# matt-graham/auxiliary-pm-mcmc

Measured on AMD Instinct MI355X. Metric: MCMC iters/sec + ESS/sec on θ, GP-classif N=4096 N_imp=256, 1/2/4/8 GPU, higher is better.
Workload: dtype mixed f64/f32

## Files before the change

### auxiliary-pm-mcmc_amd/csrc/apm_host.h

```cpp
#pragma once
#include <hip/hip_runtime.h>

#include <algorithm>
#include <cstdint>
#include <cstring>
#include <functional>
#include <initializer_list>
#include <map>
#include <string>
#include <tuple>
#include <utility>
#include <vector>

#include "../../include/apm.h"
#include "apm_internal.h"

#define HIPC(x)                                                                              \
    do {                                                                                     \
        hipError_t e_ = (x);                                                                 \
        if (e_ != hipSuccess)                                                                \
            throw HipError{std::string(#x) + ": " + hipGetErrorString(e_)};                  \
    } while (0)

namespace apm_host __attribute__((visibility("hidden"))) {

struct ProfRec {
    hipEvent_t a, b;
    int kind;
    double work;
};

#define APM_ICM_Q 1.0e3

struct Edges {
    hipEvent_t gram_k = nullptr;
    hipEvent_t cholk_done = nullptr;
    hipEvent_t y2 = nullptr;
    hipEvent_t bottom_done = nullptr;
    std::vector<hipEvent_t> cholk_rel;
    std::vector<hipEvent_t> lp_panel;
    std::vector<hipEvent_t> df;
    std::vector<hipEvent_t> far;
    std::vector<hipEvent_t*> all() {
        std::vector<hipEvent_t*> v{&gram_k, &cholk_done, &y2, &bottom_done};
        for (auto* w : {&cholk_rel, &lp_panel, &df, &far})
            for (hipEvent_t& e : *w) v.push_back(&e);
        return v;
    }
};

typedef std::pair<unsigned*, int> DevList;
typedef std::map<std::tuple<int, int, int, int, int, int>, DevList> ListCache;

struct StagePin {
    int64_t B;
    size_t slots() const { return 0; }
    size_t ubufs() const { return slots() + sizeof(int64_t) * B; }
    size_t h3ok() const { return ubufs() + sizeof(int64_t) * B; }
    size_t h3post() const { return h3ok() + sizeof(int) * B; }
    size_t invok() const { return h3post() + sizeof(int) * B; }
    size_t icm() const { return invok() + 2 * sizeof(int) * B; }
    size_t bytes() const { return icm() + sizeof(double) * B; }
};
enum StageBlk {
    BLK_I3 = 0, BLK_A = 1, BLK_B = 2, BLK_CA = 3, BLK_CB = 4, BLK_SEEDS = 5, BLK_CTRS = 6,
    BLK_FIELDS = 7
};
inline size_t read_back_bytes(int64_t B) { return (sizeof(double) + 3 * sizeof(int)) * B; }

}

struct __attribute__((visibility("hidden"))) apm_ctx {
    int device = 0;
    hipStream_t stream = nullptr;
    int kind = 0, n = 0, d = 0, np = 0, nb = 0, P = 0, S = 0, sp = 0;
    int max_batch = 0, n_slots = 0, n_ubufs = 0;
    static constexpr int outer = 8, outer32 = 8;
    static constexpr int symv_tpw = 2;
    std::vector<int> slot_refs;
    std::vector<int> slot_wide;
    std::vector<int> slot_failed;
    std::vector<double*> l64_h, l64_free;
    double** l64_d = nullptr;
    double eps = 1e-8, tol = 1e-4;
    int lik = APM_LIK_PROBIT;
    int64_t max_iters = 1000;
    std::string err;
    double *X = nullptr, *y = nullptr, *theta = nullptr;
    MatB K{}, A{};
    double *Dinv = nullptr, *ldet = nullptr, *out = nullptr, *partial = nullptr;
    int64_t dstride = 0, lstride = 0, pstride = 0;
    NewtonVecs v{};
    double* vecbase = nullptr;
    double* rvec = nullptr;
    double* sympart = nullptr;
    int64_t sstride = 0;
    bool mixed = true;
    int n_refine = 3;
    double refine_tol = 1e-3;
    int *active = nullptr, *status = nullptr, *n_iter = nullptr;
    int* refining = nullptr;
    double* refine_prev = nullptr;
    int64_t n_refine_steps = 0, n_fp64_rerun = 0;
    int64_t n_icm_check = 0;
    int64_t n_guard = 0;
    double icm_q = APM_ICM_Q;
    int64_t *d_slots = nullptr, *d_ubufs = nullptr, *d_i3 = nullptr;
    char* hpin = nullptr;
    int64_t* hblk = nullptr;
    double* hth = nullptr;
    unsigned* hx = nullptr;
    unsigned* dx = nullptr;
    double *d_ca = nullptr, *d_cb = nullptr;
    uint64_t *d_seeds = nullptr, *d_ctrs = nullptr;
    double* U64 = nullptr;
    SlotSet Sl{};
    UPool Up{};
    std::vector<void*> allocs;
    bool k_full = false;
    int prof = 0;
    std::vector<hipEvent_t> evpool;
    size_t evnext = 0;
    std::vector<apm_host::ProfRec> recs;
    apm_host::ListCache tile_lists, super_lists, super_lists_solo, super_lists_ext;
    std::map<std::tuple<int, int, int, int>, apm_host::DevList> quad_lists;
    bool h3 = true;
// ... 234 lines not shown
```

### auxiliary-pm-mcmc_amd/csrc/apm_internal.h

```cpp
#pragma once
#include <string>

#include "apm_common.h"
#include "tile_lists.h"
#include "tri_index.h"

struct MatB {
    double* base;
    int64_t ld;
    int64_t cstride;
};

struct MatF {
    float* base;
    int64_t ld;
    int64_t cstride;
};

struct Live {
    const int* active;
    int* status;
};
__device__ __forceinline__ bool live_chain(const Live& lv, int b) {
    return lv.active[b] != 0 && lv.status[b] == 0;
// ... 54 lines not shown
                              const int* h3ok, hipStream_t s,
                              Planes16 pl = Planes16{nullptr, 0, 0, 0});

void launch_chol_update32(MatF A, int k0, int kc, const unsigned* tiles, int ntiles, Live live,
                          int nchains, hipStream_t s,
                          FusedDiag<float> fd = FusedDiag<float>{0, nullptr, 0, nullptr, 0, 0},
                          int hlim = 0, const int* h3ok = nullptr);
enum {
    UPD32_NEWTON = 0,
    UPD32_POST = 1,
    UPD32_NEWTON_PLANES = 2,
};
void launch_chol_update32_t128(MatF A, int k0, int kc, const unsigned* tiles, int ntiles,
                               Live live, int nchains, hipStream_t s,
                               FusedDiag<float> fd = FusedDiag<float>{0, nullptr, 0, nullptr, 0, 0},
                               int hlim = 0, const int* h3ok = nullptr, int rhs = -1,
                               int role = UPD32_NEWTON, Planes16 pl = Planes16{nullptr, 0, 0, 0});
void launch_chol_update32_q256(MatF A, int k0, int kc, const unsigned* quads, int nq, Live live,
                               int nchains, hipStream_t s, const int* h3ok, Planes16 pl,
                               int role = UPD32_NEWTON, int npan = 1, int64_t pstep = 0);
void launch_rhs_row_update32(MatF A, int k0, int kc, const unsigned* tiles, int ntiles, Live live,
                             int nchains, hipStream_t s);

void launch_symv(MatB K, const double* x, int64_t xstride, double* y, int64_t ystride,
                 double* part, int64_t pstride, int np, MatF Bf, const double* Ws,
                 int64_t wstride, Live live, int nchains, hipStream_t s, int symv_tpw = 1);
void launch_row32(MatF Bf, int64_t row, int np, double* out, int64_t ostride, Live live,
                  int nchains, hipStream_t s);
void launch_trsv_fwd32(MatF A, int J, int nb, const float* Dinv, int64_t dstride, double* r,
                       double* y, int64_t vstride, Live live, int nchains, hipStream_t s);
void launch_trsv_bwd32(MatF A, int J, const float* Dinv, int64_t dstride, double* r, double* z,
                       int64_t vstride, Live live, int nchains, hipStream_t s);
bool trsv32_mw_ok(int np);
void trsv32_mw_init();
long launch_trsv32_mw(bool fwd, MatF A, int nb, const float* Dinv, int64_t dstride,
                      const double* r, double* out, int64_t vstride, Live live, int nchains,
                      int fail_code, SpinCtl sc, hipStream_t s);
void launch_refine_check(const double* x, const double* d, int64_t vstride, int np, double tol,
                         int fail_code, int step, bool last, double* prev, int* refining,
                         const int* status, int nchains, hipStream_t s);
void launch_refine_mask(Live live, int* refining, int nchains, hipStream_t s);
void launch_refine(int mode, const double* Ws, const double* Kb, double* x, const double* Kt,
                   double* out, int64_t vstride, int np, Live live, int nchains, hipStream_t s);

enum { APM_FAM_SE = 0, APM_FAM_M32 = 1, APM_FAM_M52 = 2 };
struct KernelKind {
    int family;
    int iso;
    int bias;
    bool on_device() const { return family >= 0; }
    int64_t theta_len(int64_t d) const { return family < 0 ? 0 : (iso ? 2 : d + 1) + bias; }
};
inline KernelKind kernel_kind_of(int kind) {
    const int bias = (kind & 16) ? 1 : 0;
    switch (kind & ~16) {
        case 0: return KernelKind{APM_FAM_SE, 1, bias};
        case 1: return KernelKind{APM_FAM_SE, 0, bias};
        case 3: return KernelKind{APM_FAM_M32, 1, bias};
        case 4: return KernelKind{APM_FAM_M32, 0, bias};
        case 5: return KernelKind{APM_FAM_M52, 1, bias};
        case 6: return KernelKind{APM_FAM_M52, 0, bias};
        default: return KernelKind{-1, 0, 0};
    }
// ... 240 lines not shown
```

### auxiliary-pm-mcmc_amd/csrc/host_ctx.cpp

```cpp
#include <cmath>
#include <cstdlib>

#include "apm_host.h"

namespace {
thread_local apm_host::SkewState t_skew;
constexpr int SKEW_US_SECONDARY = 1000, SKEW_US_MAIN = 40;
}

void skew_point(hipStream_t s) {
    if (!t_skew.mode || !s) return;
    if ((t_skew.mode & 1) && (s == t_skew.s2 || s == t_skew.s3))
        launch_delay(SKEW_US_SECONDARY, s);
    else if ((t_skew.mode & 2) && s == t_skew.main)
        launch_delay(SKEW_US_MAIN, s);
}

namespace apm_host {

SkewScope::SkewScope(const apm_ctx* c) : prev(t_skew) {
    t_skew = SkewState{c->skew & 3, c->stream, c->stream2, c->stream3};
}
SkewScope::~SkewScope() { t_skew = prev; }

// ... 87 lines not shown
        c->l64_free.pop_back();
    } else {
        c->l64_h[slot] = dalloc<double>(c, c->np * c->np);
    }
}
void detach_l64(apm_ctx* c, int64_t slot) {
    if (!c->l64_h[slot]) return;
    c->l64_free.push_back(c->l64_h[slot]);
    c->l64_h[slot] = nullptr;
}
void upload_l64(apm_ctx* c) {
    HIPC(hipMemcpyAsync(c->l64_d, c->l64_h.data(), sizeof(double*) * c->n_slots,
                        hipMemcpyHostToDevice, c->stream));
}

void init_ctx(apm_ctx* c, int device, int kind, const double* X, int64_t n, int64_t d,
              int64_t ldx, const double* y, double eps, int64_t S, int64_t max_batch,
              int64_t n_slots, int64_t n_ubufs) {
    c->device = device;
    HIPC(hipSetDevice(device));
    trsv32_mw_init();
    if (const char* e = getenv("APM_MIXED")) c->mixed = atoi(e) != 0;
    if (const char* e = getenv("APM_H3")) c->h3 = atoi(e) != 0;
    if (const char* e = getenv("APM_REFINE_TOL")) c->refine_tol = atof(e);
    if (const char* e = getenv("APM_ICM_Q")) c->icm_q = std::max(0.0, atof(e));
    if (const char* e = getenv("APM_SPIN_LIMIT")) c->spin_df = c->spin_trsv = std::max(1, atoi(e));
    if (const char* e = getenv("APM_SKEW")) c->skew = std::max(0, std::min(7, atoi(e)));
    {
        int least = 0, greatest = 0;
        HIPC(hipDeviceGetStreamPriorityRange(&least, &greatest));
        HIPC(hipStreamCreateWithPriority(&c->stream, hipStreamNonBlocking, greatest));
        HIPC(hipStreamCreateWithPriority(&c->stream2, hipStreamNonBlocking, least));
        HIPC(hipStreamCreateWithPriority(&c->stream3, hipStreamNonBlocking, least));
    }
    c->kind = kind;
    c->n = (int)n;
    c->d = (int)d;
    c->np = (int)((n + 63) / 64 * 64);
    c->nb = c->np / 64;
    {
        const int np64 = (c->nb + c->outer - 1) / c->outer, np32 = (c->nb + c->outer32 - 1) / c->outer32;
        c->ev.cholk_rel.assign(np64, nullptr);
        c->ev.lp_panel.assign(np64, nullptr);
        c->ev.df.assign(np32, nullptr);
        c->ev.far.assign(np32, nullptr);
        for (hipEvent_t* e : c->ev.all()) HIPC(hipEventCreateWithFlags(e, hipEventDisableTiming));
// ... 32 lines not shown
    c->partial = dalloc<double>(c, B * c->pstride);
    const int64_t vs = np;
    c->vecbase = dalloc<double>(c, 8 * B * vs);
    c->rvec = dalloc<double>(c, 3 * B * vs);
    c->sstride = (int64_t)c->nb * c->nb * 64;
    c->sympart = dalloc<double>(c, B * c->sstride);
    c->v = NewtonVecs{c->vecbase,          c->vecbase + 1 * B * vs, c->vecbase + 2 * B * vs,
                      c->vecbase + 3 * B * vs, c->vecbase + 4 * B * vs, c->vecbase + 5 * B * vs,
                      c->vecbase + 6 * B * vs, c->vecbase + 7 * B * vs, vs};
    HIPC(hipMemset(c->vecbase, 0, sizeof(double) * 8 * B * vs));
    c->active = dalloc<int>(c, B);
    c->status = dalloc<int>(c, B);
    c->n_iter = dalloc<int>(c, B);
    c->refining = dalloc<int>(c, B);
    c->active2 = dalloc<int>(c, B);
    c->status2 = dalloc<int>(c, B);
    c->refine_prev = dalloc<double>(c, B);
    c->d_slots = dalloc<int64_t>(c, 2 * B);
    c->d_ubufs = c->d_slots + B;
    HIPC(hipHostMalloc(reinterpret_cast<void**>(&c->hpin), pin_of(c).bytes(),
                       hipHostMallocDefault));
    HIPC(hipHostMalloc(reinterpret_cast<void**>(&c->hmask), sizeof(int) * (size_t)B,
                       hipHostMallocDefault));
    HIPC(hipHostMalloc(reinterpret_cast<void**>(&c->hx), read_back_bytes(B),
                       hipHostMallocMapped | hipHostMallocCoherent));
    HIPC(hipHostGetDevicePointer(reinterpret_cast<void**>(&c->dx), c->hx, 0));
    c->h3ok = dalloc<int>(c, 3 * B);
    c->h3post = c->h3ok + B;
    c->invok = c->h3ok + 2 * B;
    c->guard = dalloc<double>(c, 6 * B);
    HIPC(hipMemset(c->guard, 0, sizeof(double) * 6 * B));
    c->guard_rows = dalloc<double>(c, B * np);
    c->icm_thr = dalloc<double>(c, B);
    if (c->mixed && c->h3) {
        c->plane_cs = 2 * np * 32 * 2 * c->outer32;
        const int npan = (c->nb + c->outer32 - 1) / c->outer32;
        const char* fl = getenv("APM_FAR_LEFT");
        if (npan > 2 && !(fl && atoi(fl) == 0)) {
            void* p = nullptr;
            if (hipMalloc(&p, sizeof(unsigned short) * npan * B * c->plane_cs) == hipSuccess) {
                c->allocs.push_back(p);
                c->planes = static_cast<unsigned short*>(p);
                c->plane_bufs = npan;
                c->far_left = true;
            } else {
                (void)hipGetLastError();
            }
// ... 77 lines not shown
```

### auxiliary-pm-mcmc_amd/csrc/host_newton.cpp

```cpp
#include "apm_host.h"

namespace apm_host {

unsigned long long* spin_words(apm_ctx* c) {
    return c->dfprog + (size_t)c->max_batch * (c->nb + 1);
}
void reset_tickets(apm_ctx* c) {
    HIPC(hipMemsetAsync(spin_words(c) + 2, 0, sizeof(unsigned long long), c->stream));
    c->ticket_base = 0;
}

namespace {

MatF b32_of(apm_ctx* c) {
    return MatF{reinterpret_cast<float*>(c->A.base), c->np, 2 * c->A.cstride};
}
SpinCtl spin_ctl(apm_ctx* c, bool trsv) {
    unsigned long long* w = spin_words(c);
    return SpinCtl{w + 2, c->ticket_base, trsv ? w + 1 : w, trsv ? c->spin_trsv : c->spin_df};
}
void trsv32(apm_ctx* c, bool fwd, MatF F, const float* D, int64_t ds, const double* r,
            double* out, Live lv, int count) {
    c->ticket_base += (unsigned long long)launch_trsv32_mw(
        fwd, F, c->nb, D, ds, r, out, c->v.vstride, lv, count, APM_STATUS_CHOL_B,
        spin_ctl(c, true), c->stream);
}
int64_t plane_step(apm_ctx* c) { return (int64_t)c->max_batch * c->plane_cs; }
Planes16 planes_of(apm_ctx* c, int K) {
    if (!c->planes || !c->h3_now) return Planes16{nullptr, 0, 0, 0};
    return Planes16{c->planes + plane_step(c) * ((K / c->outer32) % c->plane_bufs), c->plane_cs,
                    c->plane_cs / 2, c->np};
}
float* dinv32_of(apm_ctx* c) { return reinterpret_cast<float*>(c->Dinv); }

void tracked_update32(apm_ctx* c, MatF M, int k0, int kc, int i0, int R, int j0, int jend,
                      int count, int fuse_k = -1, int fail_code = 0, hipStream_t st = nullptr,
                      Planes16 pl = Planes16{nullptr, 0, 0, 0}, int jext = -1) {
    if (!st) st = c->stream;
    if (i0 < j0) i0 = j0;
    if (update_tile_count(i0, R, j0, jend) <= 0) return;
    const auto tl = tile_list(c, i0, R, j0, jend, Gap{0, 0});
    if (tl.second <= 0) return;
    FusedDiag<float> fd{0, nullptr, 0, nullptr, 0, 0};
    if (fuse_k >= 0)
        fd = FusedDiag<float>{1, dinv32_of(c), 2 * c->dstride, c->ldet, c->lstride, fail_code};
    const bool outer = kc >= 2 && jend - j0 >= 2 && (fuse_k < 0 || (i0 == fuse_k && j0 == fuse_k));
    const int rhs = R > c->nb || jext > 0 ? c->nb : -1;
    const bool quad =
// ... 132 lines not shown
            feed_chol_k(c);
            trsv32(c, true, F, D, ds, r1, r2, lr, count);
            feed_chol_k(c);
            trsv32(c, false, F, D, ds, r2, r3, lr, count);
        } else {
            for (int J = 0; J < nb; ++J)
                launch_trsv_fwd32(F, J, nb, D, ds, r1, r2, vs, lr, count, s);
            for (int J = nb - 1; J >= 0; --J)
                launch_trsv_bwd32(F, J, D, ds, r2, r3, vs, lr, count, s);
        }
        launch_refine(2, nullptr, nullptr, c->v.z, nullptr, r3, vs, np, lr, count, s);
        const bool last = it + 1 == c->n_refine;
        launch_refine_check(c->v.z, r3, vs, np, c->refine_tol, APM_STATUS_CHOL_B, it, last,
                            c->refine_prev, c->refining, c->status, count, s);
        ++c->n_refine_steps;
        if (last) break;
        read_back(c, {RB{c->refining, (int)sizeof(int) * count, ref_h.data()}});
        bool any = false;
        for (int b = 0; b < count; ++b) any |= ref_h[b] != 0;
        if (!any) break;
    }
}

}

void newton(apm_ctx* c, int count, std::vector<int>& st_h, bool mixed, int live0) {
    const Live lv = live_of(c);
    c->live_n = live0;
    launch_refine(3, nullptr, nullptr, nullptr, nullptr, c->v.f, c->v.vstride, c->np, lv, count,
                  c->stream);
    std::vector<int> act(count, 1);
    const int64_t rrow = c->np;
    int64_t it = 0;
    for (; it < c->max_iters; ++it) {
        c->cholk_quota = 1 << 30;
        if (c->newton_last > 0 && c->cholk_next >= 0 && c->cholk_next < c->nb) {
            const int left = (c->nb - c->cholk_next + c->outer - 1) / c->outer;
            const int its = std::max<int>(1, c->newton_last - (int)it);
            c->cholk_quota = (left + its - 1) / its;
        }
        launch_newton_prep(c->lik, c->v, c->y, c->n, c->np, lv, count, c->stream);
        if (mixed) {
            launch_symv(c->K, c->v.b, c->v.vstride, c->v.Kb, c->v.vstride, c->sympart, c->sstride,
                        c->np, b32_of(c), c->v.Ws, c->v.vstride, lv, count, c->stream,
                        c->symv_tpw);
        } else if (c->k_full) {
            launch_gemv(c->K, c->v.b, c->v.vstride, c->v.Kb, c->v.vstride, c->np, lv, count,
                        c->stream);
        } else {
            launch_symv(c->K, c->v.b, c->v.vstride, c->v.Kb, c->v.vstride, c->sympart, c->sstride,
                        c->np, MatF{}, nullptr, 0, lv, count, c->stream, c->symv_tpw);
        }
        if (mixed) {
            newton_solve32(c, count);
        } else {
            launch_form_B(c->K, c->A, c->v, c->np, lv, count, c->stream);
            chol_factor(c, c->A, 0, c->nb, c->nb + 1, c->nb, APM_STATUS_CHOL_B, count);
            for (int J = c->nb - 1; J >= 0; --J)
                launch_trsv_lt_step(c->A, J, rrow, c->Dinv, c->dstride, c->v.z, c->v.vstride, lv,
                                    count, c->stream);
        }
        launch_newton_update(c->v, c->np, lv, count, c->stream);
        if (mixed || !c->k_full)
            launch_symv(c->K, c->v.a, c->v.vstride, c->v.fnew, c->v.vstride, c->sympart,
                        c->sstride, c->np, MatF{}, nullptr, 0, lv, count, c->stream, c->symv_tpw);
        else
            launch_gemv(c->K, c->v.a, c->v.vstride, c->v.fnew, c->v.vstride, c->np, lv, count,
                        c->stream);
        launch_newton_check(c->v, c->n, c->np, c->tol, c->active, c->status, c->n_iter, count,
                            c->stream);
        read_back(c, {RB{c->active, (int)sizeof(int) * count, act.data()},
                      RB{c->status, (int)sizeof(int) * count, st_h.data()}});
        int live = 0;
        for (int b = 0; b < count; ++b) live += (act[b] != 0 && st_h[b] == 0);
        if (!live) break;
        c->live_n = live;
    }
    if (mixed) c->newton_last = (int)std::min<int64_t>(it + 1, c->max_iters);
    c->cholk_quota = 1 << 30;
    bool changed = false;
    for (int b = 0; b < count; ++b)
        if (act[b] != 0 && st_h[b] == 0) {
            st_h[b] = APM_STATUS_MAXITER;
            changed = true;
        }
    if (changed)
        HIPC(hipMemcpyAsync(c->status, st_h.data(), sizeof(int) * count, hipMemcpyHostToDevice,
                            c->stream));
}

void newton_is(apm_ctx* c, int count, std::vector<int>& st_h) {
    newton(c, count, st_h, c->mixed, count);
    if (!c->mixed) return;
    std::vector<int> redo;
    for (int b = 0; b < count; ++b)
// ... 21 lines not shown
```

### auxiliary-pm-mcmc_amd/csrc/newton.hip

```cpp
#include "apm_internal.h"

template <int LIK>
__global__ __launch_bounds__(256) void k_newton_prep(NewtonVecs v, const double* __restrict__ y,
                                                     int n, int np, Live live) {
    const int b = blockIdx.y;
    if (!live_chain(live, b)) return;
    const int i = blockIdx.x * 256 + threadIdx.x;
    if (i >= np) return;
    const int64_t o = b * v.vstride + i;
    double W = 0.0, Ws = 0.0, bb = 0.0;
    if (i < n) {
        const double f = v.f[o], yi = y[i];
        const LikGW l = lik_grad_W<LIK>(f, yi);
        W = l.W;
        Ws = sqrt(W);
        bb = W * f + l.grad;
    }
    v.W[o] = W;
    v.Ws[o] = Ws;
    v.b[o] = bb;
}

void launch_newton_prep(int lik, NewtonVecs v, const double* y, int n, int np, Live live,
                        int nchains, hipStream_t s) {
// ... 48 lines not shown
    } else {
        const int tj = t - ntri;
        const int64_t r0 = (int64_t)nb * 64;
        const double* Kbv = v.Kb + b * v.vstride;
        for (int e = tid; e < 4096; e += 256) {
            const int rr = e >> 6, c = tj * 64 + (e & 63);
            Ab[(r0 + rr) * A.ld + c] = (rr == 0) ? Ws[c] * Kbv[c] : 0.0;
        }
    }
}

void launch_form_B(MatB K, MatB A, NewtonVecs v, int np, Live live, int nchains, hipStream_t s) {
    const int nb = np / 64;
    APM_LAUNCH(k_form_B, dim3(nb * (nb + 1) / 2 + nb, nchains), dim3(256), 0, s, K, A, v,
                       nb, live);
}

__global__ __launch_bounds__(256) void k_newton_update(NewtonVecs v, int np, Live live) {
    const int b = blockIdx.y;
    if (!live_chain(live, b)) return;
    const int i = blockIdx.x * 256 + threadIdx.x;
    if (i >= np) return;
    const int64_t o = b * v.vstride + i;
    v.a[o] = v.b[o] - v.Ws[o] * v.z[o];
}

void launch_newton_update(NewtonVecs v, int np, Live live, int nchains, hipStream_t s) {
    APM_LAUNCH(k_newton_update, dim3((np + 255) / 256, nchains), dim3(256), 0, s, v, np,
                       live);
}

__global__ __launch_bounds__(256) void k_newton_check(NewtonVecs v, int n, int np, double tol,
                                                      int* active, const int* status,
                                                      int* n_iter) {
    const int b = blockIdx.x;
    if (active[b] == 0 || status[b] != 0) return;
    __shared__ double red[4];
    const double* fn = v.fnew + b * v.vstride;
    double* f = v.f + b * v.vstride;
    double s = 0.0;
#pragma unroll 4
    for (int i = threadIdx.x; i < n; i += 256) {
        const double d = fn[i] - f[i];
        s += d * d;
    }
    s = block_sum_d(s, red);
    __syncthreads();
// ... 350 lines not shown
```

### auxiliary-pm-mcmc_amd/csrc/newton_solve.hip

```cpp
#include "apm_internal.h"
#include "tile32.h"


__global__ __launch_bounds__(256) void k_row32(MatF Bf, int64_t row, int np, double* out,
                                               int64_t ostride, Live live) {
    const int b = blockIdx.y;
    if (!live_chain(live, b)) return;
    const int c = blockIdx.x * 256 + threadIdx.x;
    if (c < np) out[b * ostride + c] = (double)Bf.base[b * Bf.cstride + row * Bf.ld + c];
}

void launch_row32(MatF Bf, int64_t row, int np, double* out, int64_t ostride, Live live,
                  int nchains, hipStream_t s) {
    APM_LAUNCH(k_row32, dim3((np + 255) / 256, nchains), dim3(256), 0, s, Bf, row, np,
                       out, ostride, live);
}

template <int TPW>
__global__ __launch_bounds__(256) void k_symv_part(MatB K, const double* __restrict__ x,
                                                   int64_t xstride, double* __restrict__ part,
                                                   int64_t pstride, int nb, MatF Bf,
                                                   const double* __restrict__ Ws, int64_t wstride,
                                                   Live live) {
    const int b = blockIdx.y;
    if (!live_chain(live, b)) return;
    const int ntile = nb * (nb + 1) / 2;
    const int tid = threadIdx.x, lane = tid & 63, w = tid >> 6;
    const int rg = tid >> 4, cg = tid & 15;
    __shared__ double cs[4][64];
    auto load = [&](int t, d2_t (&v)[4][2]) {
        int ti, tj;
        lower_tri_index(t, ti, tj);
        const double* Kt =
            K.base + b * K.cstride + (int64_t)(ti * 64 + 4 * rg) * K.ld + tj * 64 + 4 * cg;
#pragma unroll
        for (int r = 0; r < 4; ++r) {
            v[r][0] = *reinterpret_cast<const d2_t*>(Kt + (int64_t)r * K.ld);
            v[r][1] = *reinterpret_cast<const d2_t*>(Kt + (int64_t)r * K.ld + 2);
// ... 60 lines not shown
                sc += __shfl_xor(sc, 16, 64);
                sc += __shfl_xor(sc, 32, 64);
                csum[c] = sc;
            }
            if (lane < 16) {
#pragma unroll
                for (int c = 0; c < 4; ++c) cs[w][4 * lane + c] = csum[c];
            }
            __syncthreads();
            if (tid < 64)
                pb[((int64_t)tj * nb + ti) * 64 + tid] = cs[0][tid] + cs[1][tid] + cs[2][tid] + cs[3][tid];
            if (TPW > 1) __syncthreads();
        }
        if (TPW > 1) {
#pragma unroll
            for (int r = 0; r < 4; ++r) {
                v[r][0] = vn[r][0];
                v[r][1] = vn[r][1];
            }
        }
    }
}

__global__ __launch_bounds__(256) void k_symv_reduce(const double* __restrict__ part,
                                                     int64_t pstride, int nb, double* y,
                                                     int64_t ystride, MatF Bf,
                                                     const double* __restrict__ Ws,
                                                     int64_t wstride, Live live) {
    const int b = blockIdx.y;
    if (!live_chain(live, b)) return;
    const int i = blockIdx.x * 256 + threadIdx.x;
    const int np = nb * 64;
    if (i >= np) return;
    const double* pb = part + b * pstride + (int64_t)(i >> 6) * nb * 64 + (i & 63);
    double s = 0.0;
    int tj = 0;
    for (; tj + 16 <= nb; tj += 16) {
        double v[16];
#pragma unroll
        for (int q = 0; q < 16; ++q) v[q] = pb[(int64_t)(tj + q) * 64];
#pragma unroll
        for (int q = 0; q < 16; ++q) s += v[q];
    }
    for (; tj < nb; ++tj) s += pb[(int64_t)tj * 64];
    y[b * ystride + i] = s;
    if (Bf.base) {
        float* col = Bf.base + b * Bf.cstride + (int64_t)np * Bf.ld + i;
        col[0] = (float)(Ws[b * wstride + i] * s);
        for (int r = 1; r < 64; ++r) col[(int64_t)r * Bf.ld] = 0.0f;
    }
}

void launch_symv(MatB K, const double* x, int64_t xstride, double* y, int64_t ystride,
                 double* part, int64_t pstride, int np, MatF Bf, const double* Ws,
                 int64_t wstride, Live live, int nchains, hipStream_t s, int symv_tpw) {
    const int nb = np / 64, nt = nb * (nb + 1) / 2;
    if (symv_tpw >= 4)
        APM_LAUNCH(k_symv_part<4>, dim3((nt + 3) / 4, nchains), dim3(256), 0, s, K, x,
                           xstride, part, pstride, nb, Bf, Ws, wstride, live);
    else if (symv_tpw == 2)
        APM_LAUNCH(k_symv_part<2>, dim3((nt + 1) / 2, nchains), dim3(256), 0, s, K, x,
                           xstride, part, pstride, nb, Bf, Ws, wstride, live);
    else
        APM_LAUNCH(k_symv_part<1>, dim3(nt, nchains), dim3(256), 0, s, K, x, xstride,
                           part, pstride, nb, Bf, Ws, wstride, live);
    APM_LAUNCH(k_symv_reduce, dim3((np + 255) / 256, nchains), dim3(256), 0, s, part,
                       pstride, nb, y, ystride, Bf, Ws, wstride, live);
}

__device__ __forceinline__ void stage_tile32(float (*T)[65], const float* src, int64_t ld) {
    for (int e = threadIdx.x; e < 4096; e += 256) T[e >> 6][e & 63] = src[(int64_t)(e >> 6) * ld + (e & 63)];
}

__global__ __launch_bounds__(256) void k_trsv_fwd32(MatF A, int J, const float* Dinv,
                                                    int64_t dstride, double* r, double* y,
                                                    int64_t vstride, Live live) {
    const int b = blockIdx.y;
    if (!live_chain(live, b)) return;
    const int I = J + blockIdx.x;
    const int tid = threadIdx.x, c = tid & 63, q = tid >> 6;
    __shared__ float T[64][65];
    __shared__ double vj[64];
    __shared__ double part[4][64];
    double* rb = r + b * vstride;
    stage_tile32(T, Dinv + b * dstride + (int64_t)J * 4096, 64);
    if (tid < 64) vj[tid] = rb[J * 64 + tid];
    __syncthreads();
    double s = 0.0;
    for (int m = q * 16; m < q * 16 + 16; ++m) s += (double)T[c][m] * vj[m];
    part[q][c] = s;
// ... 223 lines not shown
                __hip_atomic_store(ob + J * 64 + row, sum, __ATOMIC_RELAXED, __HIP_MEMORY_SCOPE_AGENT);
            }
        }
    }
    __syncthreads();
    if (t == 0 && bad) {
        live.status[b] = fail_code;
        atomicAdd(sc.timeouts, 1ull);
    }
}

bool trsv32_mw_ok(int np) { return np <= TRF_MAXNP; }

void trsv32_mw_init() {
    const int mx = (int)(sizeof(double) * (TRF_MAXNP + 4 * 64 + 64));
    (void)hipFuncSetAttribute((const void*)k_trsv32_mw<true>,
                              hipFuncAttributeMaxDynamicSharedMemorySize, mx);
    (void)hipFuncSetAttribute((const void*)k_trsv32_mw<false>,
                              hipFuncAttributeMaxDynamicSharedMemorySize, mx);
}

long launch_trsv32_mw(bool fwd, MatF A, int nb, const float* Dinv, int64_t dstride,
                      const double* r, double* out, int64_t vstride, Live live, int nchains,
                      int fail_code, SpinCtl sc, hipStream_t s) {
    const size_t lds = sizeof(double) * (nb * 64 + 4 * 64 + 64);
    const int np = nb * 64;
    const int G = TRM_G;
    APM_LAUNCH(k_nan_fill, dim3((np + 255) / 256, nchains), dim3(256), 0, s, out, vstride,
                       np, live);
    if (fwd)
        APM_LAUNCH(k_trsv32_mw<true>, dim3(nchains * G), dim3(256), lds, s, A, nb,
                           Dinv, dstride, r, out, vstride, live, fail_code, G, nchains, sc);
    else
        APM_LAUNCH(k_trsv32_mw<false>, dim3(nchains * G), dim3(256), lds, s, A, nb,
                           Dinv, dstride, r, out, vstride, live, fail_code, G, nchains, sc);
    return (long)nchains * G;
}

void launch_trsv_fwd32(MatF A, int J, int nb, const float* Dinv, int64_t dstride, double* r,
                       double* y, int64_t vstride, Live live, int nchains, hipStream_t s) {
    APM_LAUNCH(k_trsv_fwd32, dim3(nb - J, nchains), dim3(256), 0, s, A, J, Dinv, dstride,
                       r, y, vstride, live);
}

void launch_trsv_bwd32(MatF A, int J, const float* Dinv, int64_t dstride, double* r, double* z,
                       int64_t vstride, Live live, int nchains, hipStream_t s) {
    APM_LAUNCH(k_trsv_bwd32, dim3(J + 1, nchains), dim3(256), 0, s, A, J, Dinv, dstride,
                       r, z, vstride, live);
}

__global__ __launch_bounds__(256) void k_refine(int mode, const double* __restrict__ Ws,
                                                const double* __restrict__ Kb, double* x,
                                                const double* __restrict__ Kt, double* out,
                                                int64_t vstride, int np, Live live) {
    const int b = blockIdx.y;
    if (!live_chain(live, b)) return;
    const int i = blockIdx.x * 256 + threadIdx.x;
    if (i >= np) return;
    const int64_t o = b * vstride + i;
    if (mode == 0)
        out[o] = Ws[o] * x[o];
    else if (mode == 1)
        out[o] = Ws[o] * Kb[o] - x[o] - Ws[o] * Kt[o];
    else if (mode == 2)
        x[o] += out[o];
    else
        out[o] = 0.0;
}

__global__ __launch_bounds__(256) void k_refine_check(const double* __restrict__ x,
                                                      const double* __restrict__ d,
                                                      int64_t vstride, int np, double tol,
                                                      int fail_code, int step, int last,
                                                      double* prev, int* refining, Live live) {
    const int b = blockIdx.x;
    if (!live_chain(live, b)) return;
    double mx = 0.0, md = 0.0;
#pragma unroll 4
    for (int i = threadIdx.x; i < np; i += 256) {
        mx = fmax(mx, fabs(x[b * vstride + i]));
        md = fmax(md, fabs(d[b * vstride + i]));
    }
    __shared__ double sx[256], sd[256];
    sx[threadIdx.x] = mx;
    sd[threadIdx.x] = md;
    __syncthreads();
    for (int h = 128; h > 0; h >>= 1) {
        if (threadIdx.x < h) {
            sx[threadIdx.x] = fmax(sx[threadIdx.x], sx[threadIdx.x + h]);
            sd[threadIdx.x] = fmax(sd[threadIdx.x], sd[threadIdx.x + h]);
        }
        __syncthreads();
    }
    if (threadIdx.x == 0) {
        const double pm = step == 0 ? sx[0] : prev[b];
        if (sd[0] * sd[0] <= tol * tol * sx[0] * pm)
            refining[b] = 0;
        else if (last)
            live.status[b] = fail_code;
        else
            prev[b] = sd[0];
    }
}

void launch_refine_check(const double* x, const double* d, int64_t vstride, int np, double tol,
                         int fail_code, int step, bool last, double* prev, int* refining,
                         const int* status, int nchains, hipStream_t s) {
    APM_LAUNCH(k_refine_check, dim3(nchains), dim3(256), 0, s, x, d, vstride, np, tol,
                       fail_code, step, (int)last, prev, refining,
                       Live{refining, const_cast<int*>(status)});
}

__global__ void k_refine_mask(Live live, int* refining, int nchains) {
    const int b = blockIdx.x * blockDim.x + threadIdx.x;
    if (b < nchains) refining[b] = live_chain(live, b) ? 1 : 0;
}

void launch_refine_mask(Live live, int* refining, int nchains, hipStream_t s) {
    APM_LAUNCH(k_refine_mask, dim3((nchains + 255) / 256), dim3(256), 0, s, live,
                       refining, nchains);
}

void launch_refine(int mode, const double* Ws, const double* Kb, double* x, const double* Kt,
                   double* out, int64_t vstride, int np, Live live, int nchains, hipStream_t s) {
    APM_LAUNCH(k_refine, dim3((np + 255) / 256, nchains), dim3(256), 0, s, mode, Ws, Kb,
                       x, Kt, out, vstride, np, live);
}
// ... 1 lines not shown
```

Measured before the change: 140.5.

## Fuse mixed-precision Newton refinement kernels and overlap host readbacks with next launches

Adds a fused path for the mixed-precision Newton solve. The residual computation is folded into the symv reduce, the NaN-fill is folded into preceding kernels, and the update, check and next-t computation are merged into one refine_step kernel. Per-step convergence flags go to mapped host memory, so the host can launch a guessed number of refinement rounds, speculatively issue the K·a symv, and read flags without blocking copies. Active/status readback now overlaps the next iteration's head kernels. The cost is extra speculative work when the guess overshoots, plus added complexity in the host/device handshake.

```diff
diff --git a/auxiliary-pm-mcmc_amd/csrc/apm_host.h b/auxiliary-pm-mcmc_amd/csrc/apm_host.h
--- a/auxiliary-pm-mcmc_amd/csrc/apm_host.h
+++ b/auxiliary-pm-mcmc_amd/csrc/apm_host.h
@@ -37,12 +37,13 @@
     hipEvent_t cholk_done = nullptr;
     hipEvent_t y2 = nullptr;
     hipEvent_t bottom_done = nullptr;
+    hipEvent_t host_wait = nullptr;
     std::vector<hipEvent_t> cholk_rel;
     std::vector<hipEvent_t> lp_panel;
     std::vector<hipEvent_t> df;
     std::vector<hipEvent_t> far;
     std::vector<hipEvent_t*> all() {
-        std::vector<hipEvent_t*> v{&gram_k, &cholk_done, &y2, &bottom_done};
+        std::vector<hipEvent_t*> v{&gram_k, &cholk_done, &y2, &bottom_done, &host_wait};
         for (auto* w : {&cholk_rel, &lp_panel, &df, &far})
             for (hipEvent_t& e : *w) v.push_back(&e);
         return v;
@@ -67,6 +68,7 @@
     BLK_FIELDS = 7
 };
 inline size_t read_back_bytes(int64_t B) { return (sizeof(double) + 3 * sizeof(int)) * B; }
+inline size_t refine_hist_bytes(int64_t B, int steps) { return sizeof(int) * B * steps; }
 
 }
 
@@ -102,6 +104,8 @@
     int* refining = nullptr;
     double* refine_prev = nullptr;
     int64_t n_refine_steps = 0, n_fp64_rerun = 0;
+    bool newton_fused = true;
+    int refine_rounds_last = 0;
     int64_t n_icm_check = 0;
     int64_t n_guard = 0;
     double icm_q = APM_ICM_Q;
diff --git a/auxiliary-pm-mcmc_amd/csrc/apm_internal.h b/auxiliary-pm-mcmc_amd/csrc/apm_internal.h
--- a/auxiliary-pm-mcmc_amd/csrc/apm_internal.h
+++ b/auxiliary-pm-mcmc_amd/csrc/apm_internal.h
@@ -100,11 +100,17 @@
 void launch_rhs_row_update32(MatF A, int k0, int kc, const unsigned* tiles, int ntiles, Live live,
                              int nchains, hipStream_t s);
 
+struct SymvRes {
+    const double *Ws, *Kb, *x;
+    double *res, *nan1, *nan2;
+    int64_t vstride;
+};
 void launch_symv(MatB K, const double* x, int64_t xstride, double* y, int64_t ystride,
                  double* part, int64_t pstride, int np, MatF Bf, const double* Ws,
-                 int64_t wstride, Live live, int nchains, hipStream_t s, int symv_tpw = 1);
+                 int64_t wstride, Live live, int nchains, hipStream_t s, int symv_tpw = 1,
+                 const SymvRes* res = nullptr);
 void launch_row32(MatF Bf, int64_t row, int np, double* out, int64_t ostride, Live live,
-                  int nchains, hipStream_t s);
+                  int nchains, hipStream_t s, double* nan = nullptr);
 void launch_trsv_fwd32(MatF A, int J, int nb, const float* Dinv, int64_t dstride, double* r,
                        double* y, int64_t vstride, Live live, int nchains, hipStream_t s);
 void launch_trsv_bwd32(MatF A, int J, const float* Dinv, int64_t dstride, double* r, double* z,
@@ -113,10 +119,17 @@
 void trsv32_mw_init();
 long launch_trsv32_mw(bool fwd, MatF A, int nb, const float* Dinv, int64_t dstride,
                       const double* r, double* out, int64_t vstride, Live live, int nchains,
-                      int fail_code, SpinCtl sc, hipStream_t s);
+                      int fail_code, SpinCtl sc, hipStream_t s, bool filled = false);
 void launch_refine_check(const double* x, const double* d, int64_t vstride, int np, double tol,
                          int fail_code, int step, bool last, double* prev, int* refining,
                          const int* status, int nchains, hipStream_t s);
+__device__ __forceinline__ double newton_a(double b, double ws, double z) { return b - ws * z; }
+void launch_refine_step(double* x, const double* d, const double* Ws, const double* bv, double* t,
+                        double* a, int64_t vstride, int np, double tol, int fail_code, int step,
+                        bool last, double* prev, int* refining, int* status, unsigned* hist,
+                        int nchains, hipStream_t s);
+void launch_refine_first(const double* Ws, const double* x, double* t, int64_t vstride, int np,
+                         Live live, int* refining, int nchains, hipStream_t s);
 void launch_refine_mask(Live live, int* refining, int nchains, hipStream_t s);
 void launch_refine(int mode, const double* Ws, const double* Kb, double* x, const double* Kt,
                    double* out, int64_t vstride, int np, Live live, int nchains, hipStream_t s);
diff --git a/auxiliary-pm-mcmc_amd/csrc/host_ctx.cpp b/auxiliary-pm-mcmc_amd/csrc/host_ctx.cpp
--- a/auxiliary-pm-mcmc_amd/csrc/host_ctx.cpp
+++ b/auxiliary-pm-mcmc_amd/csrc/host_ctx.cpp
@@ -133,6 +133,7 @@
     trsv32_mw_init();
     if (const char* e = getenv("APM_MIXED")) c->mixed = atoi(e) != 0;
     if (const char* e = getenv("APM_H3")) c->h3 = atoi(e) != 0;
+    if (const char* e = getenv("APM_NEWTON_FUSED")) c->newton_fused = atoi(e) != 0;
     if (const char* e = getenv("APM_REFINE_TOL")) c->refine_tol = atof(e);
     if (const char* e = getenv("APM_ICM_Q")) c->icm_q = std::max(0.0, atof(e));
     if (const char* e = getenv("APM_SPIN_LIMIT")) c->spin_df = c->spin_trsv = std::max(1, atoi(e));
@@ -211,7 +212,8 @@
                        hipHostMallocDefault));
     HIPC(hipHostMalloc(reinterpret_cast<void**>(&c->hmask), sizeof(int) * (size_t)B,
                        hipHostMallocDefault));
-    HIPC(hipHostMalloc(reinterpret_cast<void**>(&c->hx), read_back_bytes(B),
+    HIPC(hipHostMalloc(reinterpret_cast<void**>(&c->hx),
+                       read_back_bytes(B) + refine_hist_bytes(B, c->n_refine),
                        hipHostMallocMapped | hipHostMallocCoherent));
     HIPC(hipHostGetDevicePointer(reinterpret_cast<void**>(&c->dx), c->hx, 0));
     c->h3ok = dalloc<int>(c, 3 * B);
diff --git a/auxiliary-pm-mcmc_amd/csrc/host_newton.cpp b/auxiliary-pm-mcmc_amd/csrc/host_newton.cpp
--- a/auxiliary-pm-mcmc_amd/csrc/host_newton.cpp
+++ b/auxiliary-pm-mcmc_amd/csrc/host_newton.cpp
@@ -20,10 +20,10 @@
     return SpinCtl{w + 2, c->ticket_base, trsv ? w + 1 : w, trsv ? c->spin_trsv : c->spin_df};
 }
 void trsv32(apm_ctx* c, bool fwd, MatF F, const float* D, int64_t ds, const double* r,
-            double* out, Live lv, int count) {
+            double* out, Live lv, int count, bool filled = false) {
     c->ticket_base += (unsigned long long)launch_trsv32_mw(
         fwd, F, c->nb, D, ds, r, out, c->v.vstride, lv, count, APM_STATUS_CHOL_B,
-        spin_ctl(c, true), c->stream);
+        spin_ctl(c, true), c->stream, filled);
 }
 int64_t plane_step(apm_ctx* c) { return (int64_t)c->max_batch * c->plane_cs; }
 Planes16 planes_of(apm_ctx* c, int K) {
@@ -202,6 +202,76 @@
     }
 }
 
+void symv_Ka(apm_ctx* c, Live lv, int count) {
+    launch_symv(c->K, c->v.a, c->v.vstride, c->v.fnew, c->v.vstride, c->sympart, c->sstride,
+                c->np, MatF{}, nullptr, 0, lv, count, c->stream, c->symv_tpw);
+}
+
+bool newton_solve32_fused(apm_ctx* c, int count) {
+    const Live lv = live_of(c);
+    hipStream_t s = c->stream;
+    const int nb = c->nb, np = c->np, B = c->max_batch;
+    const int64_t vs = c->v.vstride, ds = 2 * c->dstride;
+    MatF F = b32_of(c);
+    float* D = dinv32_of(c);
+    double *r1 = c->rvec, *r2 = c->rvec + c->max_batch * vs, *r3 = c->rvec + 2 * c->max_batch * vs;
+    const size_t hoff = read_back_bytes(B) / sizeof(unsigned);
+    chol_range32(c, F, 0, nb, nb + 1, nb, APM_STATUS_CHOL_B, count);
+    launch_row32(F, np, np, r1, vs, lv, count, s, c->v.z);
+    feed_chol_k(c);
+    trsv32(c, false, F, D, ds, r1, c->v.z, lv, count, true);
+    launch_refine_first(c->v.Ws, c->v.z, r2, vs, np, lv, c->refining, count, s);
+    const Live lr{c->refining, c->status};
+    const SymvRes res{c->v.Ws, c->v.Kb, c->v.z, r1, r2, r3, vs};
+    const int guess = c->refine_rounds_last;
+    int done = 0, needed = 0;
+    bool ka = false;
+    for (;;) {
+        const int target = std::min(c->n_refine, std::max(done + 1, guess));
+        for (; done < target; ++done) {
+            launch_symv(c->K, r2, vs, r3, vs, c->sympart, c->sstride, np, MatF{}, nullptr, 0, lr,
+                        count, s, c->symv_tpw, &res);
+            feed_chol_k(c);
+            trsv32(c, true, F, D, ds, r1, r2, lr, count, true);
+            feed_chol_k(c);
+            trsv32(c, false, F, D, ds, r2, r3, lr, count, true);
+            launch_refine_step(c->v.z, r3, c->v.Ws, c->v.b, r2, c->v.a, vs, np, c->refine_tol,
+                               APM_STATUS_CHOL_B, done, done + 1 == c->n_refine, c->refine_prev,
+                               c->refining, c->status, c->dx + hoff + (size_t)done * B, count, s);
+        }
+        HIPC(hipEventRecord(c->ev.host_wait, s));
+        ka = guess > 0 && done >= guess;
+        if (ka) symv_Ka(c, lv, count);
+        HIPC(hipEventSynchronize(c->ev.host_wait));
+        bool finished = false;
+        while (needed < done && !finished) {
+            const volatile unsigned* h = c->hx + hoff + (size_t)needed * B;
+            ++needed;
+            ++c->n_refine_steps;
+            bool any = false;
+            for (int b = 0; b < count; ++b) any |= h[b] != 0;
+            finished = needed == c->n_refine || !any;
+        }
+        if (finished) break;
+    }
+    c->refine_rounds_last = needed;
+    return ka;
+}
+
+void newton_head(apm_ctx* c, Live lv, int count, bool mixed) {
+    launch_newton_prep(c->lik, c->v, c->y, c->n, c->np, lv, count, c->stream);
+    if (mixed) {
+        launch_symv(c->K, c->v.b, c->v.vstride, c->v.Kb, c->v.vstride, c->sympart, c->sstride,
+                    c->np, b32_of(c), c->v.Ws, c->v.vstride, lv, count, c->stream, c->symv_tpw);
+    } else if (c->k_full) {
+        launch_gemv(c->K, c->v.b, c->v.vstride, c->v.Kb, c->v.vstride, c->np, lv, count,
+                    c->stream);
+    } else {
+        launch_symv(c->K, c->v.b, c->v.vstride, c->v.Kb, c->v.vstride, c->sympart, c->sstride,
+                    c->np, MatF{}, nullptr, 0, lv, count, c->stream, c->symv_tpw);
+    }
+}
+
 }
 
 void newton(apm_ctx* c, int count, std::vector<int>& st_h, bool mixed, int live0) {
@@ -210,8 +280,11 @@
     launch_refine(3, nullptr, nullptr, nullptr, nullptr, c->v.f, c->v.vstride, c->np, lv, count,
                   c->stream);
     std::vector<int> act(count, 1);
+    const bool fused = mixed && c->newton_fused && c->n_refine > 0 && trsv32_mw_ok(c->np);
+    c->refine_rounds_last = 0;
     const int64_t rrow = c->np;
     int64_t it = 0;
+    bool head_done = false;
     for (; it < c->max_iters; ++it) {
         c->cholk_quota = 1 << 30;
         if (c->newton_last > 0 && c->cholk_next >= 0 && c->cholk_next < c->nb) {
@@ -219,19 +292,12 @@
             const int its = std::max<int>(1, c->newton_last - (int)it);
             c->cholk_quota = (left + its - 1) / its;
         }
-        launch_newton_prep(c->lik, c->v, c->y, c->n, c->np, lv, count, c->stream);
-        if (mixed) {
-            launch_symv(c->K, c->v.b, c->v.vstride, c->v.Kb, c->v.vstride, c->sympart, c->sstride,
-                        c->np, b32_of(c), c->v.Ws, c->v.vstride, lv, count, c->stream,
-                        c->symv_tpw);
-        } else if (c->k_full) {
-            launch_gemv(c->K, c->v.b, c->v.vstride, c->v.Kb, c->v.vstride, c->np, lv, count,
-                        c->stream);
-        } else {
-            launch_symv(c->K, c->v.b, c->v.vstride, c->v.Kb, c->v.vstride, c->sympart, c->sstride,
-                        c->np, MatF{}, nullptr, 0, lv, count, c->stream, c->symv_tpw);
-        }
-        if (mixed) {
+        if (!head_done) newton_head(c, lv, count, mixed);
+        head_done = false;
+        bool have_Ka = false;
+        if (fused) {
+            have_Ka = newton_solve32_fused(c, count);
+        } else if (mixed) {
             newton_solve32(c, count);
         } else {
             launch_form_B(c->K, c->A, c->v, c->np, lv, count, c->stream);
@@ -240,17 +306,31 @@
                 launch_trsv_lt_step(c->A, J, rrow, c->Dinv, c->dstride, c->v.z, c->v.vstride, lv,
                                     count, c->stream);
         }
-        launch_newton_update(c->v, c->np, lv, count, c->stream);
-        if (mixed || !c->k_full)
-            launch_symv(c->K, c->v.a, c->v.vstride, c->v.fnew, c->v.vstride, c->sympart,
-                        c->sstride, c->np, MatF{}, nullptr, 0, lv, count, c->stream, c->symv_tpw);
-        else
+        if (!fused) launch_newton_update(c->v, c->np, lv, count, c->stream);
+        if (mixed || !c->k_full) {
+            if (!have_Ka) symv_Ka(c, lv, count);
+        } else
             launch_gemv(c->K, c->v.a, c->v.vstride, c->v.fnew, c->v.vstride, c->np, lv, count,
                         c->stream);
         launch_newton_check(c->v, c->n, c->np, c->tol, c->active, c->status, c->n_iter, count,
                             c->stream);
-        read_back(c, {RB{c->active, (int)sizeof(int) * count, act.data()},
-                      RB{c->status, (int)sizeof(int) * count, st_h.data()}});
+        if (fused && it + 1 < c->max_iters) {
+            Export e{};
+            e.src[0] = reinterpret_cast<const unsigned*>(c->active);
+            e.src[1] = reinterpret_cast<const unsigned*>(c->status);
+            e.words[0] = e.words[1] = count;
+            e.dst = c->dx;
+            launch_export(e, c->stream);
+            HIPC(hipEventRecord(c->ev.host_wait, c->stream));
+            newton_head(c, lv, count, mixed);
+            head_done = true;
+            HIPC(hipEventSynchronize(c->ev.host_wait));
+            std::memcpy(act.data(), c->hx, sizeof(int) * count);
+            std::memcpy(st_h.data(), c->hx + count, sizeof(int) * count);
+        } else {
+            read_back(c, {RB{c->active, (int)sizeof(int) * count, act.data()},
+                          RB{c->status, (int)sizeof(int) * count, st_h.data()}});
+        }
         int live = 0;
         for (int b = 0; b < count; ++b) live += (act[b] != 0 && st_h[b] == 0);
         if (!live) break;
diff --git a/auxiliary-pm-mcmc_amd/csrc/newton.hip b/auxiliary-pm-mcmc_amd/csrc/newton.hip
--- a/auxiliary-pm-mcmc_amd/csrc/newton.hip
+++ b/auxiliary-pm-mcmc_amd/csrc/newton.hip
@@ -94,7 +94,7 @@
     const int i = blockIdx.x * 256 + threadIdx.x;
     if (i >= np) return;
     const int64_t o = b * v.vstride + i;
-    v.a[o] = v.b[o] - v.Ws[o] * v.z[o];
+    v.a[o] = newton_a(v.b[o], v.Ws[o], v.z[o]);
 }
 
 void launch_newton_update(NewtonVecs v, int np, Live live, int nchains, hipStream_t s) {
diff --git a/auxiliary-pm-mcmc_amd/csrc/newton_solve.hip b/auxiliary-pm-mcmc_amd/csrc/newton_solve.hip
--- a/auxiliary-pm-mcmc_amd/csrc/newton_solve.hip
+++ b/auxiliary-pm-mcmc_amd/csrc/newton_solve.hip
@@ -3,17 +3,19 @@
 
 
 __global__ __launch_bounds__(256) void k_row32(MatF Bf, int64_t row, int np, double* out,
-                                               int64_t ostride, Live live) {
+                                               int64_t ostride, Live live, double* nan) {
     const int b = blockIdx.y;
     if (!live_chain(live, b)) return;
     const int c = blockIdx.x * 256 + threadIdx.x;
-    if (c < np) out[b * ostride + c] = (double)Bf.base[b * Bf.cstride + row * Bf.ld + c];
+    if (c >= np) return;
+    out[b * ostride + c] = (double)Bf.base[b * Bf.cstride + row * Bf.ld + c];
+    if (nan) nan[b * ostride + c] = __builtin_nan("");
 }
 
 void launch_row32(MatF Bf, int64_t row, int np, double* out, int64_t ostride, Live live,
-                  int nchains, hipStream_t s) {
+                  int nchains, hipStream_t s, double* nan) {
     APM_LAUNCH(k_row32, dim3((np + 255) / 256, nchains), dim3(256), 0, s, Bf, row, np,
-                       out, ostride, live);
+                       out, ostride, live, nan);
 }
 
 template <int TPW>
@@ -120,6 +122,40 @@
     }
 }
 
+__device__ __forceinline__ double symv_row_sum(const double* __restrict__ pb, int nb) {
+    double s = 0.0;
+    int tj = 0;
+    for (; tj + 16 <= nb; tj += 16) {
+        double v[16];
+#pragma unroll
+        for (int q = 0; q < 16; ++q) v[q] = pb[(int64_t)(tj + q) * 64];
+#pragma unroll
+        for (int q = 0; q < 16; ++q) s += v[q];
+    }
+    for (; tj < nb; ++tj) s += pb[(int64_t)tj * 64];
+    return s;
+}
+
+__device__ __forceinline__ double refine_residual(double ws, double kb, double x, double kt) {
+    return ws * kb - x - ws * kt;
+}
+
+__global__ __launch_bounds__(256) void k_symv_reduce_res(const double* __restrict__ part,
+                                                         int64_t pstride, int nb, SymvRes e,
+                                                         Live live) {
+    const int b = blockIdx.y;
+    if (!live_chain(live, b)) return;
+    const int i = blockIdx.x * 256 + threadIdx.x;
+    const int np = nb * 64;
+    if (i >= np) return;
+    const double s =
+        symv_row_sum(part + b * pstride + (int64_t)(i >> 6) * nb * 64 + (i & 63), nb);
+    const int64_t o = b * e.vstride + i;
+    e.res[o] = refine_residual(e.Ws[o], e.Kb[o], e.x[o], s);
+    e.nan1[o] = __builtin_nan("");
+    e.nan2[o] = __builtin_nan("");
+}
+
 __global__ __launch_bounds__(256) void k_symv_reduce(const double* __restrict__ part,
                                                      int64_t pstride, int nb, double* y,
                                                      int64_t ystride, MatF Bf,
@@ -130,17 +166,8 @@
     const int i = blockIdx.x * 256 + threadIdx.x;
     const int np = nb * 64;
     if (i >= np) return;
-    const double* pb = part + b * pstride + (int64_t)(i >> 6) * nb * 64 + (i & 63);
-    double s = 0.0;
-    int tj = 0;
-    for (; tj + 16 <= nb; tj += 16) {
-        double v[16];
-#pragma unroll
-        for (int q = 0; q < 16; ++q) v[q] = pb[(int64_t)(tj + q) * 64];
-#pragma unroll
-        for (int q = 0; q < 16; ++q) s += v[q];
-    }
-    for (; tj < nb; ++tj) s += pb[(int64_t)tj * 64];
+    const double s =
+        symv_row_sum(part + b * pstride + (int64_t)(i >> 6) * nb * 64 + (i & 63), nb);
     y[b * ystride + i] = s;
     if (Bf.base) {
         float* col = Bf.base + b * Bf.cstride + (int64_t)np * Bf.ld + i;
@@ -151,7 +178,8 @@
 
 void launch_symv(MatB K, const double* x, int64_t xstride, double* y, int64_t ystride,
                  double* part, int64_t pstride, int np, MatF Bf, const double* Ws,
-                 int64_t wstride, Live live, int nchains, hipStream_t s, int symv_tpw) {
+                 int64_t wstride, Live live, int nchains, hipStream_t s, int symv_tpw,
+                 const SymvRes* res) {
     const int nb = np / 64, nt = nb * (nb + 1) / 2;
     if (symv_tpw >= 4)
         APM_LAUNCH(k_symv_part<4>, dim3((nt + 3) / 4, nchains), dim3(256), 0, s, K, x,
@@ -162,8 +190,12 @@
     else
         APM_LAUNCH(k_symv_part<1>, dim3(nt, nchains), dim3(256), 0, s, K, x, xstride,
                            part, pstride, nb, Bf, Ws, wstride, live);
-    APM_LAUNCH(k_symv_reduce, dim3((np + 255) / 256, nchains), dim3(256), 0, s, part,
-                       pstride, nb, y, ystride, Bf, Ws, wstride, live);
+    if (res)
+        APM_LAUNCH(k_symv_reduce_res, dim3((np + 255) / 256, nchains), dim3(256), 0, s, part,
+                   pstride, nb, *res, live);
+    else
+        APM_LAUNCH(k_symv_reduce, dim3((np + 255) / 256, nchains), dim3(256), 0, s, part,
+                   pstride, nb, y, ystride, Bf, Ws, wstride, live);
 }
 
 __device__ __forceinline__ void stage_tile32(float (*T)[65], const float* src, int64_t ld) {
@@ -433,12 +465,13 @@
 
 long launch_trsv32_mw(bool fwd, MatF A, int nb, const float* Dinv, int64_t dstride,
                       const double* r, double* out, int64_t vstride, Live live, int nchains,
-                      int fail_code, SpinCtl sc, hipStream_t s) {
+                      int fail_code, SpinCtl sc, hipStream_t s, bool filled) {
     const size_t lds = sizeof(double) * (nb * 64 + 4 * 64 + 64);
     const int np = nb * 64;
     const int G = TRM_G;
-    APM_LAUNCH(k_nan_fill, dim3((np + 255) / 256, nchains), dim3(256), 0, s, out, vstride,
-                       np, live);
+    if (!filled)
+        APM_LAUNCH(k_nan_fill, dim3((np + 255) / 256, nchains), dim3(256), 0, s, out, vstride,
+                   np, live);
     if (fwd)
         APM_LAUNCH(k_trsv32_mw<true>, dim3(nchains * G), dim3(256), lds, s, A, nb,
                            Dinv, dstride, r, out, vstride, live, fail_code, G, nchains, sc);
@@ -472,7 +505,7 @@
     if (mode == 0)
         out[o] = Ws[o] * x[o];
     else if (mode == 1)
-        out[o] = Ws[o] * Kb[o] - x[o] - Ws[o] * Kt[o];
+        out[o] = refine_residual(Ws[o], Kb[o], x[o], Kt[o]);
     else if (mode == 2)
         x[o] += out[o];
     else
@@ -514,6 +547,84 @@
     }
 }
 
+__global__ __launch_bounds__(1024) void k_refine_step(double* x, const double* __restrict__ d,
+                                                     const double* __restrict__ Ws,
+                                                     const double* __restrict__ bv, double* t,
+                                                     double* a, int64_t vstride, int np,
+                                                     double tol, int fail_code, int step,
+                                                     int last, double* prev, int* refining,
+                                                     Live live, unsigned* hist) {
+    const int b = blockIdx.x;
+    if (!live_chain(live, b)) {
+        if (threadIdx.x == 0) {
+            hist[b] = (unsigned)refining[b];
+            __threadfence_system();
+        }
+        return;
+    }
+    double mx = 0.0, md = 0.0;
+    for (int i = threadIdx.x; i < np; i += 1024) {
+        const int64_t o = b * vstride + i;
+        const double di = d[o], xn = x[o] + di, ws = Ws[o];
+        x[o] = xn;
+        t[o] = ws * xn;
+        a[o] = newton_a(bv[o], ws, xn);
+        mx = fmax(mx, fabs(xn));
+        md = fmax(md, fabs(di));
+    }
+    __shared__ double sx[1024], sd[1024];
+    sx[threadIdx.x] = mx;
+    sd[threadIdx.x] = md;
+    __syncthreads();
+    for (int h = 512; h > 0; h >>= 1) {
+        if (threadIdx.x < h) {
+            sx[threadIdx.x] = fmax(sx[threadIdx.x], sx[threadIdx.x + h]);
+            sd[threadIdx.x] = fmax(sd[threadIdx.x], sd[threadIdx.x + h]);
+        }
+        __syncthreads();
+    }
+    if (threadIdx.x == 0) {
+        const double pm = step == 0 ? sx[0] : prev[b];
+        int still = 1;
+        if (sd[0] * sd[0] <= tol * tol * sx[0] * pm)
+            refining[b] = still = 0;
+        else if (last)
+            live.status[b] = fail_code;
+        else
+            prev[b] = sd[0];
+        hist[b] = (unsigned)still;
+        __threadfence_system();
+    }
+}
+
+void launch_refine_step(double* x, const double* d, const double* Ws, const double* bv, double* t,
+                        double* a, int64_t vstride, int np, double tol, int fail_code, int step,
+                        bool last, double* prev, int* refining, int* status, unsigned* hist,
+                        int nchains, hipStream_t s) {
+    APM_LAUNCH(k_refine_step, dim3(nchains), dim3(1024), 0, s, x, d, Ws, bv, t, a, vstride, np, tol,
+               fail_code, step, (int)last, prev, refining, Live{refining, status}, hist);
+}
+
+__global__ __launch_bounds__(256) void k_refine_first(const double* __restrict__ Ws,
+                                                      const double* __restrict__ x, double* t,
+                                                      int64_t vstride, int np, Live live,
+                                                      int* refining) {
+    const int b = blockIdx.y;
+    const bool lv = live_chain(live, b);
+    if (blockIdx.x == 0 && threadIdx.x == 0) refining[b] = lv ? 1 : 0;
+    if (!lv) return;
+    const int i = blockIdx.x * 256 + threadIdx.x;
+    if (i >= np) return;
+    const int64_t o = b * vstride + i;
+    t[o] = Ws[o] * x[o];
+}
+
+void launch_refine_first(const double* Ws, const double* x, double* t, int64_t vstride, int np,
+                         Live live, int* refining, int nchains, hipStream_t s) {
+    APM_LAUNCH(k_refine_first, dim3((np + 255) / 256, nchains), dim3(256), 0, s, Ws, x, t, vstride,
+               np, live, refining);
+}
+
 void launch_refine_check(const double* x, const double* d, int64_t vstride, int np, double tol,
                          int fail_code, int step, bool last, double* prev, int* refining,
                          const int* status, int nchains, hipStream_t s) {
```

Result: no change. 140.9 (median of 4 runs) (+0.3%).
